# choi403/ALG

Measured on AMD Instinct MI355X. Metric: frames/sec (whole node) CogVideoX-5B-I2V 49f x 50-step ALG, higher is better.
Workload: dtype bf16; 1 GPU; BASELINE config 2: CogVideoX-5B-I2V bf16, 49 frames @ 480x720, 50 steps, ALG interval down_up (resize_factor 0.25, interval [0, 0.04]), guidance 6.0; one video per GPU; layers=42, dit_sample_forwards=12, parallelism=dp1

## Files before the change

alg_amd/_lib.py:

```python
from __future__ import annotations

import ctypes
from collections import OrderedDict
import os
from ctypes import POINTER, Structure, byref, c_char_p, c_float, c_int, c_int32, c_int64, c_void_p

import torch

_HERE = os.path.dirname(os.path.abspath(__file__))
LIB_PATH = os.environ.get("ALG_HIP_LIB") or os.path.join(_HERE, "libalg_hip.so")

ALG_F32, ALG_BF16 = 0, 1
ACT_NONE, ACT_GELU_TANH, ACT_SILU = 0, 1, 2
GEMM_BIAS_PER_ROW, GEMM_PERMUTE_COLS, GEMM_GATE_F32, GEMM_GATE_SEG_STRIDE = 1, 4, 8, 16
GEMM_B_PACKED11 = 32

EXPORTS = (
    "alg_version", "alg_last_error", "alg_reload_env", "alg_down_up", "alg_gaussian_blur", "alg_cfg_ddim_step", "alg_gemm_bf16", "alg_gemm_bf16_pair", "alg_gemm_bf16_pair_qk", "alg_pack_b_p11", "alg_pack_b_p11_bytes",
    "alg_flash_attn_d64", "alg_layernorm_modulate", "alg_layernorm_modulate_fp8", "alg_qk_norm_rope", "alg_patchify", "alg_unpatchify",
    "alg_timestep_embedding", "alg_cfg_combine", "alg_lincomb", "alg_unipc_update", "alg_concat_cast", "alg_flash_attn_d128", "alg_layernorm_mod_f32", "alg_layernorm_mod_f32_fp8", "alg_rmsnorm_rope",
    "alg_wan_modulation", "alg_patchify3d", "alg_unpatchify3d", "alg_timestep_embedding_f32", "alg_linear_f32",
    "alg_gelu_erf", "alg_layernorm_modulate_seg", "alg_headnorm_rope", "alg_masked_mean", "alg_silu", "alg_gemm_fp8", "alg_quantize_fp8_rows",
    "alg_conv_cl_bf16", "alg_vae_groupnorm_workspace", "alg_vae_groupnorm_stats", "alg_vae_spatial_norm", "alg_vae_upsample",
    "alg_vae_pack_latent", "alg_vae_unpack_video", "alg_vae_group_norm", "alg_vae_pad", "alg_vae_repitch",
    "alg_vae_unpack_planes", "alg_rms_norm_rows", "alg_softmax_hilo", "alg_flash_attn_d128_ex", "alg_flash_attn_d128_dual", "alg_rope_half", "alg_patchify_t", "alg_unpatchify_t", "alg_qk_norm_rope_scaled", "alg_flash_attn_d64_ex", "alg_embed_rows", "alg_t5_layernorm", "alg_attn_bias", "alg_mul_bf16", "alg_quick_gelu",
    "alg_lowpass_tables_bytes", "alg_lowpass_tables_build", "alg_down_up_workspace_bytes", "alg_gaussian_blur_workspace_bytes",
    "alg_flash_attn_d64_workspace_bytes", "alg_calib_mfma_bf16", "alg_wall_clock_khz", "alg_attn_clock_tap",
    "alg_flash_attn_d128_fp8", "alg_quantize_fp8_khead", "alg_quantize_fp8_vt", "alg_rmsnorm_rope_fp8", "alg_headnorm_rope_fp8",
)
_RET_I64 = ("alg_vae_groupnorm_workspace", "alg_lowpass_tables_bytes", "alg_down_up_workspace_bytes",
            "alg_gaussian_blur_workspace_bytes", "alg_flash_attn_d64_workspace_bytes", "alg_pack_b_p11_bytes")


class AlgHipError(RuntimeError):
    pass


class GemmArgs(Structure):
    _fields_ = [
        ("A", c_void_p), ("B", c_void_p), ("C", c_void_p), ("bias", c_void_p), ("R", c_void_p), ("gate", c_void_p),
        ("lda", c_int64), ("ldb", c_int64), ("ldc", c_int64), ("ldr", c_int64),
        ("strideA", c_int64), ("strideB", c_int64), ("strideC", c_int64), ("strideR", c_int64),
        ("strideGate", c_int64),
        ("M", c_int32), ("N", c_int32), ("K", c_int32), ("batch", c_int32),
        ("seg_split", c_int32), ("act", c_int32), ("flags", c_int32),
        ("gate_seg_stride", c_int64), ("perm_col0", c_int32), ("conv_cin_log2", c_int32),
        ("a_scale", c_void_p), ("b_scale", c_void_p), ("strideAScale", c_int64), ("strideBScale", c_int64),
        ("conv_wp", c_int32), ("conv_hpwp", c_int32), ("conv_kw", c_int32), ("reserved1", c_int32),
    ]


class QkNormRopeArgs(Structure):
    _fields_ = [("wq", c_void_p), ("bq", c_void_p), ("wk", c_void_p), ("bk", c_void_p), ("cos_tab", c_void_p),
                ("sin_tab", c_void_p), ("heads", c_int32), ("text_len", c_int32), ("eps", c_float),
                ("q_scale", c_float)]


class VaeGeom(Structure):
    _fields_ = [(n, c_int32) for n in ("frames", "H", "W", "C", "first_len", "seg_len", "lat_first_single", "lat_rate",
                                       "lat_scale", "lat_h", "lat_w")]


_lib = None


def build_library(verbose=False):
    import subprocess

    src = os.path.join(_HERE, "csrc")
    r = subprocess.run(["make", "-C", src, "-j8"], capture_output=True, text=True)
    if verbose or r.returncode != 0:
        print(r.stdout[-4000:])
        print(r.stderr[-4000:])
    if r.returncode != 0:
        raise AlgHipError("building libalg_hip.so failed (see output above)")
    return LIB_PATH


# ... 59 lines not shown
    lib.alg_vae_groupnorm_workspace.argtypes = [POINTER(VaeGeom)]
    lib.alg_vae_groupnorm_stats.argtypes = [c_void_p, POINTER(VaeGeom), c_float, c_void_p, c_void_p, c_void_p]
    lib.alg_vae_spatial_norm.argtypes = [c_void_p] * 6 + [POINTER(VaeGeom), c_int, c_void_p]
    lib.alg_vae_group_norm.argtypes = [c_void_p] * 5 + [POINTER(VaeGeom), c_int, c_void_p]
    lib.alg_vae_pad.argtypes = [c_void_p, c_void_p] + [c_int] * 4 + [c_void_p]
    lib.alg_vae_repitch.argtypes = [c_void_p, c_void_p] + [c_int] * 6 + [c_void_p]
    lib.alg_vae_unpack_planes.argtypes = [c_void_p, c_void_p] + [c_int] * 4 + [c_void_p]
    lib.alg_embed_rows.argtypes = [c_void_p, c_void_p, c_void_p, c_int64, c_int, c_int, c_void_p]
    lib.alg_t5_layernorm.argtypes = [c_void_p, c_void_p, c_void_p, c_int64, c_int, c_float, c_void_p]
    lib.alg_attn_bias.argtypes = [c_void_p] * 7 + [c_int, c_int, c_int, c_int, c_int64, c_int64, c_float, c_int, c_void_p]
    lib.alg_quick_gelu.argtypes = [c_void_p, c_int64, c_void_p]
    lib.alg_mul_bf16.argtypes = [c_void_p, c_void_p, c_void_p, c_int64, c_void_p]
    lib.alg_vae_upsample.argtypes = [c_void_p, c_void_p] + [c_int] * 6 + [c_void_p]
    lib.alg_vae_pack_latent.argtypes = [c_void_p, c_int64, c_int64, c_void_p, c_int, c_int, c_int, c_int, c_float, c_void_p]
    lib.alg_vae_unpack_video.argtypes = [c_void_p, c_void_p, c_int, c_int, c_int, c_int, c_void_p]
    lib.alg_quantize_fp8_rows.argtypes = [c_void_p, c_int64, c_void_p, c_void_p, c_int64, c_int, c_void_p]
    lib.alg_timestep_embedding_f32.argtypes = [c_void_p, c_void_p, c_int, c_int, c_void_p]
    lib.alg_linear_f32.argtypes = [c_void_p] * 6 + [c_int] * 4 + [c_void_p]
    lib.alg_gelu_erf.argtypes = [c_void_p, c_int64, c_void_p]
    lib.alg_unipc_update.argtypes = [c_void_p] * 5 + [c_int64] + [c_float] * 6 + [c_void_p]
    lib.alg_gemm_bf16.argtypes = [POINTER(GemmArgs), c_void_p]
    lib.alg_gemm_bf16_pair.argtypes = [POINTER(GemmArgs), POINTER(GemmArgs), c_void_p]
    lib.alg_gemm_bf16_pair_qk.argtypes = [POINTER(GemmArgs), POINTER(GemmArgs), POINTER(QkNormRopeArgs), c_void_p]
    lib.alg_flash_attn_d64.argtypes = [c_void_p, c_void_p, c_void_p, c_void_p, c_int, c_int, c_int, c_int64, c_int64,
                                       c_int64, c_int64, c_int64, c_int64, c_float, c_void_p]
    lib.alg_layernorm_modulate.argtypes = [c_void_p, c_void_p, c_void_p, c_void_p, c_void_p, c_void_p, c_int64, c_int,
                                           c_int, c_int, c_int64, c_int64, c_int, c_float, c_void_p]
    lib.alg_layernorm_modulate_fp8.argtypes = [c_void_p] * 7 + [c_int64, c_int, c_int, c_int, c_int64, c_int, c_float, c_void_p]
    lib.alg_qk_norm_rope.argtypes = [c_void_p, c_void_p, c_void_p, c_void_p, c_void_p, c_void_p, c_void_p, c_int,
                                     c_int, c_int, c_int, c_float, c_void_p]
    lib.alg_qk_norm_rope_scaled.argtypes = [c_void_p] * 7 + [c_int, c_int, c_int, c_int, c_float, c_float, c_void_p]
    lib.alg_flash_attn_d64_ex.argtypes = [c_void_p, c_void_p, c_void_p, c_void_p, c_int, c_int, c_int, c_int64, c_int64,
                                          c_int64, c_int64, c_int64, c_int64, c_float, c_int, c_void_p, c_int64, c_void_p]
    lib.alg_patchify.argtypes = [c_void_p, c_int64, POINTER(c_void_p), c_void_p, c_int, c_int, c_int, c_int, c_int,
                                 c_int, c_void_p]
    lib.alg_unpatchify.argtypes = [c_void_p, c_void_p, c_int, c_int, c_int, c_int, c_int, c_int, c_void_p]
    lib.alg_patchify_t.argtypes = [c_void_p, c_int64, POINTER(c_void_p), c_void_p] + [c_int] * 7 + [c_void_p]
    lib.alg_unpatchify_t.argtypes = [c_void_p, c_void_p] + [c_int] * 7 + [c_void_p]
    lib.alg_timestep_embedding.argtypes = [c_void_p, c_void_p, c_int, c_int, c_int, c_void_p]
    lib.alg_calib_mfma_bf16.argtypes = [c_void_p, c_int, ctypes.c_uint, c_int, c_void_p, c_void_p]
    lib.alg_attn_clock_tap.argtypes = [c_void_p, c_int]
    for name in EXPORTS:
        fn = getattr(lib, name)
        if name == "alg_attn_clock_tap":
            fn.restype = None
        elif name not in ("alg_version", "alg_last_error", "alg_reload_env"):
# ... 600 lines not shown
        _check(lib.alg_gemm_bf16(ctypes.byref(args), _stream()), "alg_gemm_bf16")


def gemm_pair(first, second):
    lib = load_library()
    a, fa = gemm_args(*first[0], **first[1])
    b, fb = gemm_args(*second[0], **second[1])
    if fa or fb:
        raise AlgHipError("gemm_pair takes bf16 problems")
    _check(lib.alg_gemm_bf16_pair(ctypes.byref(a), ctypes.byref(b), _stream()), "alg_gemm_bf16_pair")


def gemm_pair_qk(first, second, wq, bq, wk, bk, cos, sin, heads, text_len, eps, q_scale=1.0):
    lib = load_library()
    a, fa = gemm_args(*first[0], **first[1])
    b, fb = gemm_args(*second[0], **second[1])
    if fa or fb:
        raise AlgHipError("gemm_pair_qk takes bf16 problems")
    ptrs = [t.data_ptr() if t is not None else None for t in (wq, bq, wk, bk, cos, sin)]
    e = QkNormRopeArgs(*ptrs, heads, text_len, float(eps), float(q_scale))
    _check(lib.alg_gemm_bf16_pair_qk(ctypes.byref(a), ctypes.byref(b), ctypes.byref(e), _stream()), "alg_gemm_bf16_pair_qk")


def quantize_fp8_rows(x, q, scale, rows, K, x_rstride=None, x_off=0, q_off=0, scale_off=0):
    x_rstride = K if x_rstride is None else x_rstride
    _check(load_library().alg_quantize_fp8_rows(_p(x, x_off), x_rstride, _p(q, q_off), _p(scale, scale_off), rows, K,
                                                _stream()), "alg_quantize_fp8_rows")
    return q, scale


ATTN_Q_PRESCALED = 1


def flash_attn_d64(q, k, vt, o, batch, heads, S, q_bstride, q_rstride, vt_bstride, vt_rstride, o_bstride, o_rstride,
                   scale, q_off=0, k_off=0, q_prescaled=False):
    lib = load_library()
    flags = ATTN_Q_PRESCALED if q_prescaled else 0
    wsb = int(lib.alg_flash_attn_d64_workspace_bytes(batch, heads, S, flags))
    ws = scratch(o, wsb, "attn_d64")
    _check(lib.alg_flash_attn_d64_ex(c_void_p(q.data_ptr() + 2 * q_off), c_void_p(k.data_ptr() + 2 * k_off), _ptr(vt),
                                     _ptr(o), batch, heads, S, q_bstride, q_rstride, vt_bstride, vt_rstride, o_bstride,
                                     o_rstride, float(scale), flags, _ptr(ws), wsb, _stream()),
           "alg_flash_attn_d64")


def layernorm_modulate(x, y, weight, bias, scale, shift, mod_bstride, batch, rows, D, seg_split, eps,
# ... 43 lines not shown
```

alg_amd/csrc/gemm.hip:

```cpp
#include <stdlib.h>

#include "common.h"

namespace alg {
constexpr int BM = 256, BN = 256;
int launch_gemm_p6(const alg_gemm_args* a, int m_tiles, int n_tiles, int64_t nwg, hipStream_t s);
int launch_gemm_p9(const alg_gemm_args* a, int m_tiles, int n_tiles, int64_t nwg, hipStream_t s);
int launch_gemm_p9_pair(const alg_gemm_args* a, int m_tiles_a, int n_tiles_a, const alg_gemm_args* b, int m_tiles_b, int n_tiles_b,
                        hipStream_t s);
int launch_gemm_p9_pair_qk(const alg_gemm_args* a, int m_tiles_a, int n_tiles_a, const alg_gemm_args* b, int m_tiles_b, int n_tiles_b,
                           const alg_qk_norm_rope_args* e, hipStream_t s);
int launch_gemm_p10(const alg_gemm_args* a, int m_tiles, int n_tiles, int64_t nwg, hipStream_t s);
int launch_gemm_p10_pair(const alg_gemm_args* a, int m_tiles_a, int n_tiles_a, const alg_gemm_args* b, int m_tiles_b, int n_tiles_b,
                         hipStream_t s);
int launch_gemm_p10_pair_qk(const alg_gemm_args* a, int m_tiles_a, int n_tiles_a, const alg_gemm_args* b, int m_tiles_b, int n_tiles_b,
                            const alg_qk_norm_rope_args* e, hipStream_t s);
int launch_gemm_p11(const alg_gemm_args* a, int m_tiles, int n_tiles, int64_t nwg, hipStream_t s);
int launch_gemm_p6_fp8(const alg_gemm_args* a, int m_tiles, int n_tiles, int64_t nwg, hipStream_t s);
int launch_gemm_p9_fp8(const alg_gemm_args* a, int m_tiles, int n_tiles, int64_t nwg, hipStream_t s);
int launch_gemm_p6_conv(const alg_gemm_args* a, int m_tiles, int n_tiles, int64_t nwg, hipStream_t s);
static int gemm_pipe() { return opt(OPT_GEMM_PIPE); }
static bool asm_pipe() { return gemm_pipe() == 9 || gemm_pipe() == 10; }
}

using namespace alg;

static int gemm_entry(const alg_gemm_args* a, void* stream, bool fp8, bool validate_only = false) {
  if (!a || !a->A || !a->B || !a->C) {
    set_error("alg_gemm_bf16: null argument");
    return ALG_EINVAL;
  }
  if (a->M <= 0 || a->N <= 0 || a->K <= 0 || a->batch <= 0) {
    set_error("alg_gemm_bf16: bad shape M=%d N=%d K=%d batch=%d", a->M, a->N, a->K, a->batch);
    return ALG_EINVAL;
  }
  if (a->K % (fp8 ? 128 : 64) != 0) {
    set_error("alg_gemm_%s: K=%d must be a multiple of %d", fp8 ? "fp8" : "bf16", a->K, fp8 ? 128 : 64);
    return ALG_EINVAL;
  }
  const int al = fp8 ? 16 : 8;
// ... 148 lines not shown
      ((uintptr_t)e->cos_tab & 15) || ((uintptr_t)e->sin_tab & 15) || ((uintptr_t)a->C & 15)) {
    set_error("alg_gemm_bf16_pair_qk: pointers must be 16-byte aligned");
    return ALG_EINVAL;
  }
  if (a->N != 2 * e->heads * 64 || a->ldc != a->N || a->strideC != (int64_t)a->M * a->N || (a->flags & ALG_GEMM_PERMUTE_COLS) ||
      a->R || a->act != ALG_ACT_NONE) {
    set_error("alg_gemm_bf16_pair_qk: qk must be a plain GEMM onto the contiguous [batch][S][2][heads][64] tensor (N=%d heads=%d ldc=%lld)",
              a->N, e->heads, (long long)a->ldc);
    return ALG_EINVAL;
  }
  const bool fused = asm_pipe() && pair_eligible(a) && pair_eligible(b) && e->heads % 4 == 0 &&
                     !(a->bias && (a->flags & ALG_GEMM_BIAS_PER_ROW));
  if (fused) {
    const int64_t ta = (int64_t)((a->M + BM - 1) / BM) * ((a->N + BN - 1) / BN) * a->batch;
    const int64_t tb = (int64_t)((b->M + BM - 1) / BM) * ((b->N + BN - 1) / BN) * b->batch;
    if (ta + tb <= 0x7fffffff)
      return (gemm_pipe() == 10 ? launch_gemm_p10_pair_qk : launch_gemm_p9_pair_qk)(a, (a->M + BM - 1) / BM, (a->N + BN - 1) / BN, b, (b->M + BM - 1) / BM, (b->N + BN - 1) / BN, e,
                                    (hipStream_t)stream);
  }
  rc = alg_gemm_bf16_pair(a, b, stream);
  if (rc != ALG_OK) return rc;
  return alg_qk_norm_rope_scaled(a->C, e->wq, e->bq, e->wk, e->bk, e->cos_tab, e->sin_tab, a->batch, a->M, e->heads, e->text_len,
                                 e->eps, e->q_scale, stream);
}

extern "C" int alg_gemm_fp8(const alg_gemm_args* a, void* stream) { return gemm_entry(a, stream, true); }

extern "C" int alg_conv_cl_bf16(const void* x, const void* w, const void* bias, const void* res, void* y, int frames,
                                int Hp, int Wp, int Cin, int Cout, int kt, int mode, void* stream) {
  const bool pair = mode == ALG_CONV_PAIR, down = mode == ALG_CONV_STRIDE2;
  if (frames <= 0 || Hp < 3 || Wp < 3 || (kt != 1 && kt != 3) || Cin < 64 || (Cin & (Cin - 1)) || Cout <= 0 || (Cout & 3) ||
      mode < 0 || mode > ALG_CONV_STRIDE2 || (pair && (((Hp * Wp) & 1) || Cout > 128)) ||
      (down && (kt != 1 || (Hp & 1) || (Wp & 1)))) {
    set_error("alg_conv_cl_bf16: bad shape frames=%d Hp=%d Wp=%d Cin=%d Cout=%d kt=%d (Cin a power of two >= 64, Cout %% 4 == 0)",
              frames, Hp, Wp, Cin, Cout, kt);
    return ALG_EINVAL;
  }
  alg_gemm_args a = {};
  a.A = x, a.B = w, a.C = y, a.bias = bias, a.R = res;
  const int vox = pair ? 2 : 1, kw = pair ? 4 : 3;
  a.lda = (int64_t)vox * Cin, a.ldb = (int64_t)kt * 3 * kw * Cin, a.ldc = (int64_t)vox * Cout, a.ldr = a.ldc;
  a.strideA = (int64_t)Hp * Wp * Cin, a.strideB = 0, a.strideC = (int64_t)Hp * Wp * Cout, a.strideR = a.strideC;
  a.M = Hp * Wp / vox, a.N = vox * Cout, a.K = kt * 3 * kw * Cin, a.batch = frames;
  a.act = ALG_ACT_NONE;
  a.conv_cin_log2 = __builtin_ctz((unsigned)Cin), a.conv_wp = Wp, a.conv_hpwp = Hp * Wp, a.conv_kw = kw;
  if (down) {
// ... 8 lines not shown
```

alg_amd/csrc/gemm_kernel.h:

```cpp
#pragma once
#include <stdlib.h>

#include <type_traits>

#include "common.h"
#include "qk_norm_rope.h"
#ifdef ALG_P9_LOOP_INC
#include ALG_P9_LOOP_INC
#else
#include "gemm_p9_loop.inc"
#endif
#include "gemm_p9_fp8_loop.inc"
#ifdef ALG_P11_LOOP_INC
#include ALG_P11_LOOP_INC
#else
#include "gemm_p11_loop.inc"
#endif
#ifdef ALG_P10_LOOP_INC
#include ALG_P10_LOOP_INC
#else
#include "gemm_p10_loop.inc"
#endif

#ifndef ALG_FP8_MX
// ... 65 lines not shown
    return x * __builtin_amdgcn_rcpf(1.0f + __builtin_amdgcn_exp2f(x * fmaf(k2, x * x, k1)));
  }
  if (act == ALG_ACT_SILU) {
    return x * __builtin_amdgcn_rcpf(1.0f + __builtin_amdgcn_exp2f(-1.4426950408889634f * x));
  }
  return x;
}

__device__ __forceinline__ void unpack4(const uint2 v, float (&f)[4]) {
  f[0] = __uint_as_float(v.x << 16);
  f[1] = __uint_as_float(v.x & 0xffff0000u);
  f[2] = __uint_as_float(v.y << 16);
  f[3] = __uint_as_float(v.y & 0xffff0000u);
}

struct GemmNoPair {};
struct GemmPairArgs {
  alg_gemm_args p;
  int m_tiles, n_tiles, group_m;
};
struct GemmPairQkArgs : GemmPairArgs {
  QkNormRope qe;
};
template <int PAIR> struct GemmPairT { typedef GemmNoPair type; };
template <> struct GemmPairT<1> { typedef GemmPairArgs type; };
template <> struct GemmPairT<2> { typedef GemmPairQkArgs type; };
template <int ACT, bool RES, int PIPE, int WNW = 4, bool FP8 = false, bool CONV = false, int PAIR = 0>
__global__ __launch_bounds__((PIPE == 11 ? 1 : 2) * WNW * 64) void gemm_bf16_kernel(
    const alg_gemm_args p1, int m_tiles1, int n_tiles1, int group_m1, const typename GemmPairT<PAIR>::type pr) {
  constexpr bool P9 = PIPE == 9 || PIPE == 10 || PIPE == 11;
  constexpr bool M16 = PIPE == 10 || PIPE == 11;
  constexpr bool P11 = PIPE == 11;
  constexpr int WMW = P11 ? 1 : 2;
  constexpr int MT = BM / WMW / 32;
  static_assert(!PAIR || (P9 && !P11 && !RES && ACT == ALG_ACT_NONE), "the pair launch is built for the plain schedule-9 / 10 kernels");
  static_assert(!FP8 || PIPE == 6 || PIPE == 9, "the fp8 operands are built on the ping-pong schedule and on schedule 9");
  static_assert(!CONV || (PIPE == 6 && !FP8), "the convolution addressing is built on the bf16 ping-pong schedule");
  typedef typename std::conditional<FP8, uint8_t, bf16_t>::type elem_t;
  constexpr int EPS = 16 / (int)sizeof(elem_t);
  constexpr int GEMM_THREADS = WMW * WNW * 64;
  constexpr int NT = BN / WNW / 32;
  static_assert(PIPE == 0 || PIPE == 6 || PIPE == 7 || PIPE == 8 || P9,
                "schedules built: 0 (2-stage ring), 6 (ping-pong), 7 (4-wave interleaved), 8 (4-wave BK = 32 ring), 9 / 10 (asm loops)");
  static_assert((PIPE == 7 || PIPE == 8 || PIPE == 9 || PIPE == 10) == (WNW == 2) && P11 == (WNW == 4 && WMW == 1),
                "PIPE 7 / 8 / 9 / 10 are the 2 x 2 4-wave layouts, 11 the 1 x 4 one, the others run 8 waves");
  static_assert(!P11 || (!FP8 && !CONV), "schedule 11 takes bf16 plain GEMM addressing with a packed B");
  static_assert(!P9 || !CONV, "schedules 9 / 10 take plain GEMM addressing (bf16, or e4m3 on 9 since round 4)");
  constexpr bool BK64 = true;
  constexpr bool PP = PIPE == 6;
  constexpr int BK = FP8 ? 128 : 64;
  constexpr int NSTAGE = 2;
  constexpr int ROW_BYTES = BK * (int)sizeof(elem_t);
  constexpr int SLOTS = ROW_BYTES / 16;
  constexpr int TILE_BYTES = BM * ROW_BYTES;
  constexpr int STAGE_BYTES = 2 * TILE_BYTES;
  constexpr int LD_PER_OP = TILE_BYTES / (GEMM_THREADS * 16);
  constexpr int ROWS_PER_LD = GEMM_THREADS / SLOTS;
  static_assert(NSTAGE * STAGE_BYTES == GEMM_LDS, "ring must fill the 128 KiB LDS budget");

  extern __shared__ __attribute__((aligned(16))) char smem[];
  const int tid = threadIdx.x;
  const int lane = tid & 63;
  const int wave = __builtin_amdgcn_readfirstlane(tid >> 6);
  const int wm = wave / WNW, wn = wave % WNW;

  constexpr int abl = 0;
#ifdef ALG_GEMM_TAP
  uint64_t tap_loop = 0, tap_tiles = 0;
  const uint64_t tap_c0 = __builtin_readcyclecounter(), tap_r0 = wall_clock64();
#endif
  group_m1 &= 0xffff;
  const int total1 = m_tiles1 * n_tiles1 * p1.batch;
  auto do_tile = [&](const int wg_in) __attribute__((always_inline)) {
  bool second = false;
  if constexpr (PAIR) second = wg_in >= total1;
  const alg_gemm_args& p = [&]() -> const alg_gemm_args& {
    if constexpr (PAIR) return second ? pr.p : p1;
    else return p1;
  }();
  int m_tiles = m_tiles1, n_tiles = n_tiles1, group_m = group_m1, wg = wg_in;
  if constexpr (PAIR) {
    if (second) m_tiles = pr.m_tiles, n_tiles = pr.n_tiles, group_m = pr.group_m, wg = wg_in - total1;
  }
  const int tiles = m_tiles * n_tiles;
  const int b = wg / tiles;
  int t = wg - b * tiles;
  const int grp = t / (group_m * n_tiles);
  const int first_m = grp * group_m;
  const int gsize = min(m_tiles - first_m, group_m);
  t -= grp * group_m * n_tiles;
  const int m0 = (first_m + t % gsize) * BM;
  const int n0 = (t / gsize) * BN;

  const elem_t* A = (const elem_t*)p.A + (int64_t)b * p.strideA;
  const elem_t* B = (const elem_t*)p.B + (int64_t)b * p.strideB;

  const int srow = tid / SLOTS;
  const int sw_src = !BK64 ? ((tid >> 4) & 3) : ((tid >> 4) & 7);
  const int sslot = (tid & (SLOTS - 1)) ^ sw_src;
  const elem_t* a_src[LD_PER_OP];
  const elem_t* b_src[LD_PER_OP];
#pragma unroll
  for (int i = 0; i < LD_PER_OP; ++i) {
    const int r = i * ROWS_PER_LD + srow;
// ... 578 lines not shown
  const bool perm = p.flags & ALG_GEMM_PERMUTE_COLS;
  const int64_t gate_seg = (p.flags & ALG_GEMM_GATE_SEG_STRIDE) ? p.gate_seg_stride : p.N;
  const bool gate_f32 = RES && p.gate && (p.flags & ALG_GEMM_GATE_F32);
  bf16_t* Cb = (bf16_t*)p.C + (int64_t)b * p.strideC;
  const int ldc = (int)p.ldc, ldr = (int)p.ldr;
  const int col0 = perm ? p.perm_col0 : 0;
  const bool n_vec = (p.N & 3) == 0 && (col0 & 15) == 0;
  auto blk_row = [&](int mt) { return PP ? (mt >> 1) * 128 + wm * 64 + (mt & 1) * 32 : wm * (MT * 32) + mt * 32; };
  auto blk_col = [&](int nt) { return PP ? nt * 128 + wn * 32 : wn * (NT * 32) + nt * 32; };
  auto quad_row = [](int q, int ln_) { return M16 ? 16 * (q >> 1) + (ln_ & 15) : (ln_ & 31); };
  auto quad_col = [](int q, int ln_) { return M16 ? 16 * (q & 1) + 4 * (ln_ >> 4) : 8 * q + 4 * (ln_ >> 5); };
  auto rq = [](int q) { return M16 ? q >> 1 : 0; };
  auto cq = [](int q) { return M16 ? q & 1 : q; };
  constexpr int NRQ = M16 ? 2 : 1, NCQ = M16 ? 2 : 4;
  if constexpr (PP || PIPE == 8 || P9) {
    const bool staged = staged_epilogue() && ((!RES && ACT == ALG_ACT_NONE) || !(bias && bias_row));
    int lane_e = lane, l31_e = l31, h2_e = h2;
    if constexpr (P9) {
      int z = 0;
      asm volatile("" : "+s"(z));
      lane_e = __builtin_amdgcn_mbcnt_hi(~0u, __builtin_amdgcn_mbcnt_lo(~0u, z));
      l31_e = lane_e & 31, h2_e = lane_e >> 5;
    }
    if (staged) {
      char* const my = smem + wave * (MT * NT * 2048);
      constexpr bool NT_OUTER = FP8 && PIPE == 9 && RES;
      uint2 bcol[NT_OUTER ? 1 : NT][4];
      float4 scol[FP8 && !NT_OUTER ? NT : 1][FP8 && !NT_OUTER ? 4 : 1];
      float brow4[MT][NRQ], a_sc4[MT];
      if constexpr (!NT_OUTER)
#pragma unroll
      for (int nt = 0; nt < NT; ++nt)
#pragma unroll
        for (int g = 0; g < NCQ; ++g) {
          const int n = n0 + blk_col(nt) + (M16 ? quad_col(g, lane_e) : 8 * g + 4 * h2_e);
          const int nc = n < p.N ? n : 0;
          if constexpr (BIAS_EARLY) bcol[nt][g] = bcol_early[nt][g];
          else bcol[nt][g] = (bias && !bias_row) ? *(const uint2*)(bias + nc) : make_uint2(0u, 0u);
          if constexpr (FP8) scol[nt][g] = *(const float4*)(p.b_scale + (int64_t)b * p.strideBScale + nc);
        }
#pragma unroll
      for (int mt = 0; mt < MT; ++mt) {
#pragma unroll
        for (int r = 0; r < NRQ; ++r) {
          const int row = m0 + blk_row(mt) + quad_row(2 * r, lane_e);
          const int rowc = row < p.M ? row : p.M - 1;
// ... 462 lines not shown
                if (gate_f32) {
                  x = bf2f(R[rowc * ldr + nn]) +
                      ((const float*)p.gate)[(int64_t)b * p.strideGate + (seg1 ? gate_seg : 0) + nn] * x;
                } else {
                  const float gg = gate ? bf2f(gate[(seg1 ? gate_seg : 0) + nn]) : 1.0f;
                  x = bf2f(R[rowc * ldr + nn]) + rbf(gg * x);
                }
              }
              const int nj = nn + col0;
              const int nc = perm ? ((nj & ~12) | ((nj & 4) << 1) | ((nj & 8) >> 1)) : nn;
              Cb[row * ldc + nc] = f2bf(x);
            }
          }
        }
      }
    });
  };
#ifndef ALG_EPI_STAGED_ONLY
  static_for<MT>([&](auto mt_c) { epilogue_band(mt_c); });
#endif
  };

  int total_wg = total1;
  if constexpr (PAIR) total_wg += pr.m_tiles * pr.n_tiles * pr.p.batch;
  for (int L = blockIdx.x; L < total_wg; L += gridDim.x) {
    const int xcd = L & 7, q = total_wg >> 3, r = total_wg & 7;
    const int wg = (xcd < r ? xcd * (q + 1) : r * (q + 1) + (xcd - r) * q) + (L >> 3);
    if (L != (int)blockIdx.x) __syncthreads();
    do_tile(wg);
  }
#ifdef ALG_GEMM_TAP
  if (threadIdx.x == 0 && blockIdx.x < 1024) {
    uint64_t* t = gemm_tap_buf + blockIdx.x * 4;
    t[0] = __builtin_readcyclecounter() - tap_c0, t[1] = wall_clock64() - tap_r0, t[2] = tap_loop, t[3] = tap_tiles;
  }
#endif
}

inline unsigned gemm_grid(int64_t nwg) {
  static std::atomic<int> cus{0};
  int n = cus.load();
  if (n == 0) {
    hipDeviceProp_t prop;
    int dev = 0;
    n = (hipGetDevice(&dev) == hipSuccess && hipGetDeviceProperties(&prop, dev) == hipSuccess) ? prop.multiProcessorCount : 256;
    n &= ~7;
    if (n < 8) n = 8;
// ... 55 lines not shown
```

alg_amd/csrc/gemm_p11.hip:

```cpp
#include "gemm_kernel.h"

namespace alg {
int launch_gemm_p11(const alg_gemm_args* a, int m_tiles, int n_tiles, int64_t nwg, hipStream_t s) {
  return launch_gemm<11, 4>(a, m_tiles, n_tiles, nwg, s);
}

__global__ __launch_bounds__(256) void pack_b_p11_kernel(const bf16_t* __restrict__ w, uint4* __restrict__ out, int N, int K, int64_t ldb,
                                                          int64_t total) {
  const int64_t i = (int64_t)blockIdx.x * 256 + threadIdx.x;
  if (i >= total) return;
  const int lane = (int)(i & 63);
  const int f = (int)((i >> 6) & 7), wv = (int)((i >> 9) & 3);
  const int64_t tile = i >> 11;
  const int nkt = K / 64;
  const int kt = (int)(tile % nkt);
  const int64_t nt = tile / nkt;
  const int n = (int)(nt * 256) + wv * 64 + (f & 3) * 16 + (lane & 15);
  const int k = kt * 64 + (f >> 2) * 32 + (lane >> 4) * 8;
  uint4 v = make_uint4(0u, 0u, 0u, 0u);
  if (n < N) v = *(const uint4*)(w + (int64_t)n * ldb + k);
  out[i] = v;
}
}

using namespace alg;

extern "C" int64_t alg_pack_b_p11_bytes(int N, int K) {
// ... 19 lines not shown
```

alg_amd/transformer_cogvideox.py:

```python
from __future__ import annotations

import math
import os
from dataclasses import dataclass, asdict
from typing import Optional

import torch

from . import _lib


@dataclass
class CogVideoXTransformerConfig:

    num_attention_heads: int = 48
    attention_head_dim: int = 64
    in_channels: int = 32
    out_channels: int = 16
    num_layers: int = 42
    time_embed_dim: int = 512
    text_embed_dim: int = 4096
    max_text_seq_length: int = 226
    sample_width: int = 90
    sample_height: int = 60
# ... 30 lines not shown
    FP8_WEIGHTS = ("wqk", "wv", "wo", "wf1", "wf2")

    def __init__(self, config: CogVideoXTransformerConfig, weights: dict, device="cuda", fp8=False):
        cfg = self.config = config
        self.device = torch.device(device)
        if self.device.type != "cuda":
            raise _lib.AlgHipError("CogVideoXTransformer3DModel runs on the GPU only (HIP kernels, no CPU fallback)")
        if cfg.attention_head_dim != 64:
            raise _lib.AlgHipError("the attention kernel is specialised for head_dim 64")
        if cfg.ofs_embed_dim is not None and cfg.ofs_embed_dim != cfg.time_embed_dim:
            raise _lib.AlgHipError("ofs_embed_dim must equal time_embed_dim (emb = emb + ofs_emb)")
        D = cfg.inner_dim
        if D % 512:
            raise _lib.AlgHipError("inner_dim must be a multiple of 512 (LayerNorm kernel tiling)")
        self.fp8 = bool(fp8)
        if self.fp8:
            self._check_fp8_shapes()
        self.fuse_quant = True
        _lib.load_library()
        self.attn_prescale = True
        self.pair_qkv = True
        self.fuse_qk_norm = False
        self.packed_weights = True
        self._sincos = {}
        dev = self.device
        w = weights
        p = cfg.patch_size
        self.p_t = cfg.patch_size_t or 1
        self.k_patch = cfg.in_channels * p * p * self.p_t
        if self.k_patch % 64 or cfg.text_embed_dim % 64 or cfg.time_embed_dim % 64:
            raise _lib.AlgHipError("GEMM K dimensions must be multiples of 64")
        self.w_patch = _bf(w["patch_embed.proj.weight"].reshape(D, self.k_patch), dev)
        self.b_patch = _bf(w["patch_embed.proj.bias"], dev)
        self.w_text = _bf(w["patch_embed.text_proj.weight"], dev)
        self.b_text = _bf(w["patch_embed.text_proj.bias"], dev)
        self.pos_emb = _bf(w["patch_embed.pos_embedding"][0], dev) if cfg.use_learned_positional_embeddings else None
        self.w_t1 = _bf(w["time_embedding.linear_1.weight"], dev)
        self.b_t1 = _bf(w["time_embedding.linear_1.bias"], dev)
        self.w_t2 = _bf(w["time_embedding.linear_2.weight"], dev)
        self.b_t2 = _bf(w["time_embedding.linear_2.bias"], dev)
        if cfg.ofs_embed_dim is not None:
            self.w_o1, self.b_o1 = _bf(w["ofs_embedding.linear_1.weight"], dev), _bf(w["ofs_embedding.linear_1.bias"], dev)
            self.w_o2, self.b_o2 = _bf(w["ofs_embedding.linear_2.weight"], dev), _bf(w["ofs_embedding.linear_2.bias"], dev)

        def reorder6(t):
            c = t.chunk(6, dim=0)
# ... 7 lines not shown
            for nm in ("norm1", "norm2"):
                mw.append(reorder6(w[b + nm + ".linear.weight"]))
                mb.append(reorder6(w[b + nm + ".linear.bias"]))
                L[nm + "_w"] = _bf(w[b + nm + ".norm.weight"], dev)
                L[nm + "_b"] = _bf(w[b + nm + ".norm.bias"], dev)
            L["wqk"] = _bf(torch.cat([w[b + "attn1.to_q.weight"], w[b + "attn1.to_k.weight"]], dim=0), dev)
            L["bqk"] = _bf(torch.cat([w[b + "attn1.to_q.bias"], w[b + "attn1.to_k.bias"]], dim=0), dev)
            L["wv"] = _bf(w[b + "attn1.to_v.weight"], dev)
            L["bv"] = _bf(w[b + "attn1.to_v.bias"], dev)
            for nm in ("norm_q", "norm_k"):
                L[nm + "_w"] = _bf(w[b + "attn1." + nm + ".weight"], dev)
                L[nm + "_b"] = _bf(w[b + "attn1." + nm + ".bias"], dev)
            L["wo"] = _bf(w[b + "attn1.to_out.0.weight"], dev)
            L["bo"] = _bf(w[b + "attn1.to_out.0.bias"], dev)
            L["wf1"] = _bf(w[b + "ff.net.0.proj.weight"], dev)
            L["bf1"] = _bf(w[b + "ff.net.0.proj.bias"], dev)
            L["wf2"] = _bf(w[b + "ff.net.2.weight"], dev)
            L["bf2"] = _bf(w[b + "ff.net.2.bias"], dev)
            if self.fp8:
                self._quantize_layer(L, drop_bf16=True)
            else:
                for nm in ("wo", "wf1", "wf2"):
                    L["p" + nm] = _lib.PackedB(L[nm])
            self.layers.append(L)
        ow, ob = w["norm_out.linear.weight"], w["norm_out.linear.bias"]
        sh_w, sc_w = ow.chunk(2, dim=0)
        sh_b, sc_b = ob.chunk(2, dim=0)
        mw.append(torch.cat([sh_w, sh_w, sc_w, sc_w], dim=0))
        mb.append(torch.cat([sh_b, sh_b, sc_b, sc_b], dim=0))
        self.w_mod = _bf(torch.cat(mw, dim=0), dev)
        self.b_mod = _bf(torch.cat(mb, dim=0), dev)
        self.mod_cols = self.w_mod.shape[0]
        self.norm_final_w = _bf(w["norm_final.weight"], dev)
        self.norm_final_b = _bf(w["norm_final.bias"], dev)
        self.norm_out_w = _bf(w["norm_out.norm.weight"], dev)
        self.norm_out_b = _bf(w["norm_out.norm.bias"], dev)
        self.w_out = _bf(w["proj_out.weight"], dev)
        self.b_out = _bf(w["proj_out.bias"], dev)
        self._ws = {}
        self._rope_cache = {}
        self.profile = None

    def _check_fp8_shapes(self):
        cfg = self.config
        D, F4 = cfg.inner_dim, cfg.ff_inner_mult * cfg.inner_dim
        if D % 128 or F4 % 128:
# ... 228 lines not shown
            emb, osin, o1, oemb = (torch.empty(N, E, device=self.device, dtype=torch.bfloat16) for _ in range(4))
            G(ws["t1"], self.w_t2, emb, N, E, E, E, E, E, bias=self.b_t2)
            ofs_v = ofs.to(device=self.device, dtype=torch.float32).reshape(-1)
            ofs_v = (ofs_v if ofs_v.numel() == N else ofs_v[:1].expand(N)).contiguous()
            _lib.timestep_embedding(ofs_v, osin, N, O, cfg.flip_sin_to_cos)
            G(osin, self.w_o1, o1, N, O, O, O, O, O, bias=self.b_o1, act=_lib.ACT_SILU)
            G(o1, self.w_o2, oemb, N, O, O, O, O, O, bias=self.b_o2)
            _lib.lincomb([(1.0, emb), (1.0, oemb)], torch.bfloat16, out=emb)
            _lib.silu(emb, ws["semb"])
        G(ws["semb"], self.w_mod, mod, N, self.mod_cols, E, E, E, self.mod_cols, bias=self.b_mod)

        G(ehs, self.w_text, x, T, D, cfg.text_embed_dim, cfg.text_embed_dim, cfg.text_embed_dim, D,
          bias=self.b_text, R=pos_emb, ldr=D, batch=N, strideA=T * cfg.text_embed_dim, strideC=S * D)
        _lib.patchify(lat, 0 if Bl == 1 else Fr * C * Hh * Ww, conds, ws["patches"], N, Fr, C, Hh, Ww, p, p_t)
        G(ws["patches"], self.w_patch, x, P, D, self.k_patch, self.k_patch, self.k_patch, D, bias=self.b_patch,
          R=pos_emb, ldr=D, r_off=T * D, batch=N, strideA=P * self.k_patch, strideC=S * D, c_off=T * D)

        scale = 1.0 / math.sqrt(cfg.attention_head_dim)
        prescale = self.attn_prescale
        q_scale = scale * 1.4426950408889634 if prescale else 1.0
        F4 = cfg.ff_inner_mult * D
        packed = self.packed_weights and os.environ.get("ALG_GEMM_PIPE", "10") == "10"
        wo_k, wf1_k, wf2_k = ("pwo", "pwf1", "pwf2") if packed else ("wo", "wf1", "wf2")
        for li, L in enumerate(self.layers):
            m1 = li * 12 * D
            m2 = m1 + 6 * D
            if fp8:
                self._block_fp8(L, ws, q8, q8s, N, S, T, m1, m2, cos, sin, scale, q_scale, prescale)
                continue
            TM("ln_mod", _lib.layernorm_modulate, x, y, L["norm1_w"], L["norm1_b"], mod, mod, self.mod_cols, N, S, D,
               T, cfg.norm_eps, scale_off=m1 + 2 * D, shift_off=m1)
            qk_call = ((y, L["wqk"], qk, S, 2 * D, D, D, D, 2 * D), dict(bias=L["bqk"], batch=N, strideA=S * D, strideC=S * 2 * D))
            vt_call = ((L["wv"], y, vt, D, S, D, D, D, S_pad), dict(bias=L["bv"], batch=N, strideB=S * D, strideC=D * S_pad,
                                                                   flags=_lib.GEMM_BIAS_PER_ROW | _lib.GEMM_PERMUTE_COLS))
            if self.pair_qkv and self.fuse_qk_norm:
                TM("gemm_qkv", _lib.gemm_pair_qk, qk_call, vt_call, L["norm_q_w"], L["norm_q_b"], L["norm_k_w"], L["norm_k_b"], cos, sin,
                               Hn, T, cfg.qk_norm_eps, q_scale=q_scale)
            else:
                if self.pair_qkv:
                    TM("gemm_qkv", _lib.gemm_pair, qk_call, vt_call)
                else:
                    TM("gemm_qk", G, *qk_call[0], **qk_call[1])
                    TM("gemm_vt", G, *vt_call[0], **vt_call[1])
                TM("qk_norm_rope", _lib.qk_norm_rope_, qk, L["norm_q_w"], L["norm_q_b"], L["norm_k_w"], L["norm_k_b"], cos, sin, N, S, Hn, T,
                                   cfg.qk_norm_eps, q_scale=q_scale)
            TM("attn", _lib.flash_attn_d64, qk, qk, vt, att, N, Hn, S, S * 2 * D, 2 * D, D * S_pad, S_pad, S * D, D, scale,
                                k_off=D, q_prescaled=prescale)
            TM("gemm_out", G, att, L[wo_k], x, S, D, D, D, D, D, bias=L["bo"], R=x, ldr=D, gate=mod, gate_off=m1 + 4 * D,
              strideGate=self.mod_cols, seg_split=T, batch=N, strideA=S * D, strideC=S * D, strideR=S * D)
            TM("ln_mod", _lib.layernorm_modulate, x, y, L["norm2_w"], L["norm2_b"], mod, mod, self.mod_cols, N, S, D,
               T, cfg.norm_eps, scale_off=m2 + 2 * D, shift_off=m2)
            TM("gemm_ff1", G, y, L[wf1_k], h, S, F4, D, D, D, F4, bias=L["bf1"], act=_lib.ACT_GELU_TANH, batch=N, strideA=S * D,
              strideC=S * F4)
            TM("gemm_ff2", G, h, L[wf2_k], x, S, D, F4, F4, F4, D, bias=L["bf2"], R=x, ldr=D, gate=mod, gate_off=m2 + 4 * D,
              strideGate=self.mod_cols, seg_split=T, batch=N, strideA=S * F4, strideC=S * D, strideR=S * D)

        _lib.layernorm_modulate(x, y, self.norm_final_w, self.norm_final_b, None, None, 0, N, S, D, T, cfg.norm_eps)
        mo = cfg.num_layers * 12 * D
# ... 26 lines not shown
```

include/alg_hip.h:

```cpp
#ifndef ALG_HIP_H
#define ALG_HIP_H

#include <stdint.h>

#ifdef __cplusplus
extern "C" {
#endif

#define ALG_F32 0
#define ALG_BF16 1

#define ALG_OK 0
#define ALG_EINVAL (-1)
#define ALG_ELAUNCH (-2)
#define ALG_ELIMIT (-3)

#define ALG_VERSION 110

int alg_version(void);
const char* alg_last_error(void);

void alg_reload_env(void);


// ... 57 lines not shown
  const float* b_scale;
  int64_t strideAScale, strideBScale;
  int32_t conv_wp;
  int32_t conv_hpwp;
  int32_t conv_kw;
  int32_t reserved1;
} alg_gemm_args;

int alg_gemm_bf16(const alg_gemm_args* args, void* stream);

int64_t alg_pack_b_p11_bytes(int N, int K);
int alg_pack_b_p11(const void* w, void* packed, int N, int K, int64_t ldb, void* stream);

int alg_gemm_bf16_pair(const alg_gemm_args* a, const alg_gemm_args* b, void* stream);

typedef struct alg_qk_norm_rope_args {
  const void *wq, *bq, *wk, *bk;
  const float *cos_tab, *sin_tab;
  int32_t heads, text_len;
  float eps, q_scale;
} alg_qk_norm_rope_args;
int alg_gemm_bf16_pair_qk(const alg_gemm_args* qk, const alg_gemm_args* vt, const alg_qk_norm_rope_args* e, void* stream);

int alg_gemm_fp8(const alg_gemm_args* args, void* stream);

int alg_quantize_fp8_rows(const void* x, int64_t x_rstride, void* q, float* scale, int64_t rows, int K, void* stream);

int alg_flash_attn_d64(const void* q, const void* k, const void* vt, void* o, int batch, int heads, int S,
                       int64_t q_bstride, int64_t q_rstride, int64_t vt_bstride, int64_t vt_rstride,
                       int64_t o_bstride, int64_t o_rstride, float scale, void* stream);

#define ALG_ATTN_Q_PRESCALED 1
int alg_flash_attn_d64_ex(const void* q, const void* k, const void* vt, void* o, int batch, int heads, int S,
                          int64_t q_bstride, int64_t q_rstride, int64_t vt_bstride, int64_t vt_rstride,
                          int64_t o_bstride, int64_t o_rstride, float scale, int flags, void* workspace,
                          int64_t workspace_bytes, void* stream);
int64_t alg_flash_attn_d64_workspace_bytes(int batch, int heads, int S, int flags);

int alg_flash_attn_d128(const void* q, const void* k, const void* vt, void* o, int batch, int heads, int Sq, int Skv,
                        int64_t q_bstride, int64_t q_rstride, int64_t k_bstride, int64_t k_rstride, int64_t vt_bstride,
                        int64_t vt_rstride, int64_t o_bstride, int64_t o_rstride, float scale, void* stream);

int alg_flash_attn_d128_ex(const void* q, const void* k, const void* vt, void* o, int batch, int heads, int Sq, int Skv,
                           int64_t q_bstride, int64_t q_rstride, int64_t k_bstride, int64_t k_rstride, int64_t vt_bstride,
                           int64_t vt_rstride, int64_t o_bstride, int64_t o_rstride, float scale, int kv_group, int causal,
                           void* stream);
// ... 160 lines not shown
```

Baseline: 1.501 frames/s.

## Fold QKV projections into one packed GEMM with a transposing V epilogue

Concatenates the QK and V weights into one packed-B matrix and runs a single schedule-11 GEMM over N=3D. Column tiles at or beyond n_split take a new epilogue that goes through LDS and writes V transposed and column-permuted into the vt buffer that attention reads. This replaces the paired schedule-10 QK/VT launch with the packed schedule-11 kernel and avoids reading the activation twice. In exchange it adds a complex shuffle epilogue and extra weight memory for the concatenated packed copy, and it only applies under the default pipe.

```diff
diff --git a/alg_amd/_lib.py b/alg_amd/_lib.py
--- a/alg_amd/_lib.py
+++ b/alg_amd/_lib.py
@@ -16,7 +16,7 @@
 GEMM_B_PACKED11 = 32
 
 EXPORTS = (
-    "alg_version", "alg_last_error", "alg_reload_env", "alg_down_up", "alg_gaussian_blur", "alg_cfg_ddim_step", "alg_gemm_bf16", "alg_gemm_bf16_pair", "alg_gemm_bf16_pair_qk", "alg_pack_b_p11", "alg_pack_b_p11_bytes",
+    "alg_version", "alg_last_error", "alg_reload_env", "alg_down_up", "alg_gaussian_blur", "alg_cfg_ddim_step", "alg_gemm_bf16", "alg_gemm_bf16_pair", "alg_gemm_bf16_pair_qk", "alg_gemm_bf16_split_t", "alg_pack_b_p11", "alg_pack_b_p11_bytes",
     "alg_flash_attn_d64", "alg_layernorm_modulate", "alg_layernorm_modulate_fp8", "alg_qk_norm_rope", "alg_patchify", "alg_unpatchify",
     "alg_timestep_embedding", "alg_cfg_combine", "alg_lincomb", "alg_unipc_update", "alg_concat_cast", "alg_flash_attn_d128", "alg_layernorm_mod_f32", "alg_layernorm_mod_f32_fp8", "alg_rmsnorm_rope",
     "alg_wan_modulation", "alg_patchify3d", "alg_unpatchify3d", "alg_timestep_embedding_f32", "alg_linear_f32",
@@ -54,6 +54,10 @@
     _fields_ = [("wq", c_void_p), ("bq", c_void_p), ("wk", c_void_p), ("bk", c_void_p), ("cos_tab", c_void_p),
                 ("sin_tab", c_void_p), ("heads", c_int32), ("text_len", c_int32), ("eps", c_float),
                 ("q_scale", c_float)]
+
+
+class GemmSplitTArgs(Structure):
+    _fields_ = [("Ct", c_void_p), ("ldct", c_int64), ("strideCt", c_int64), ("n_split", c_int32), ("perm_col0", c_int32)]
 
 
 class VaeGeom(Structure):
@@ -159,6 +163,7 @@
     lib.alg_gemm_bf16.argtypes = [POINTER(GemmArgs), c_void_p]
     lib.alg_gemm_bf16_pair.argtypes = [POINTER(GemmArgs), POINTER(GemmArgs), c_void_p]
     lib.alg_gemm_bf16_pair_qk.argtypes = [POINTER(GemmArgs), POINTER(GemmArgs), POINTER(QkNormRopeArgs), c_void_p]
+    lib.alg_gemm_bf16_split_t.argtypes = [POINTER(GemmArgs), POINTER(GemmSplitTArgs), c_void_p]
     lib.alg_flash_attn_d64.argtypes = [c_void_p, c_void_p, c_void_p, c_void_p, c_int, c_int, c_int, c_int64, c_int64,
                                        c_int64, c_int64, c_int64, c_int64, c_float, c_void_p]
     lib.alg_layernorm_modulate.argtypes = [c_void_p, c_void_p, c_void_p, c_void_p, c_void_p, c_void_p, c_int64, c_int,
@@ -805,6 +810,15 @@
     _check(lib.alg_gemm_bf16_pair_qk(ctypes.byref(a), ctypes.byref(b), ctypes.byref(e), _stream()), "alg_gemm_bf16_pair_qk")
 
 
+def gemm_split_t(problem, n_split, Ct, ldct, strideCt=0, perm_col0=0, ct_off=0):
+    lib = load_library()
+    a, fp8 = gemm_args(*problem[0], **problem[1])
+    if fp8:
+        raise AlgHipError("gemm_split_t takes a bf16 problem")
+    t = GemmSplitTArgs((Ct.data_ptr() + 2 * ct_off) if Ct is not None else None, ldct, strideCt, n_split, perm_col0)
+    _check(lib.alg_gemm_bf16_split_t(ctypes.byref(a), ctypes.byref(t), _stream()), "alg_gemm_bf16_split_t")
+
+
 def quantize_fp8_rows(x, q, scale, rows, K, x_rstride=None, x_off=0, q_off=0, scale_off=0):
     x_rstride = K if x_rstride is None else x_rstride
     _check(load_library().alg_quantize_fp8_rows(_p(x, x_off), x_rstride, _p(q, q_off), _p(scale, scale_off), rows, K,
diff --git a/alg_amd/csrc/gemm.hip b/alg_amd/csrc/gemm.hip
--- a/alg_amd/csrc/gemm.hip
+++ b/alg_amd/csrc/gemm.hip
@@ -16,6 +16,7 @@
 int launch_gemm_p10_pair_qk(const alg_gemm_args* a, int m_tiles_a, int n_tiles_a, const alg_gemm_args* b, int m_tiles_b, int n_tiles_b,
                             const alg_qk_norm_rope_args* e, hipStream_t s);
 int launch_gemm_p11(const alg_gemm_args* a, int m_tiles, int n_tiles, int64_t nwg, hipStream_t s);
+int launch_gemm_p11_split_t(const alg_gemm_args* a, int m_tiles, int n_tiles, int64_t nwg, const alg_gemm_split_t_args* t, hipStream_t s);
 int launch_gemm_p6_fp8(const alg_gemm_args* a, int m_tiles, int n_tiles, int64_t nwg, hipStream_t s);
 int launch_gemm_p9_fp8(const alg_gemm_args* a, int m_tiles, int n_tiles, int64_t nwg, hipStream_t s);
 int launch_gemm_p6_conv(const alg_gemm_args* a, int m_tiles, int n_tiles, int64_t nwg, hipStream_t s);
@@ -210,6 +211,50 @@
   if (rc != ALG_OK) return rc;
   return alg_qk_norm_rope_scaled(a->C, e->wq, e->bq, e->wk, e->bk, e->cos_tab, e->sin_tab, a->batch, a->M, e->heads, e->text_len,
                                  e->eps, e->q_scale, stream);
+}
+
+extern "C" int alg_gemm_bf16_split_t(const alg_gemm_args* a, const alg_gemm_split_t_args* t, void* stream) {
+  const int rc = gemm_entry(a, stream, false, true);
+  if (rc != ALG_OK) return rc;
+  if (!t) {
+    set_error("alg_gemm_bf16_split_t: null argument");
+    return ALG_EINVAL;
+  }
+  if (!(a->flags & ALG_GEMM_B_PACKED11) || (a->flags & ~ALG_GEMM_B_PACKED11) || a->R || a->gate || a->act != ALG_ACT_NONE || a->a_scale ||
+      a->b_scale || a->conv_wp || a->conv_cin_log2 || a->conv_kw) {
+    set_error("alg_gemm_bf16_split_t: takes a plain bf16 problem with a packed B (ALG_GEMM_B_PACKED11 and no other flag; no residual, gate, "
+              "activation, e4m3 scales or convolution addressing)");
+    return ALG_EINVAL;
+  }
+  if (gemm_pipe() != 10) {
+    set_error("alg_gemm_bf16_split_t: built for the default schedule only (ALG_GEMM_PIPE=%d): run the two projections as their own calls", gemm_pipe());
+    return ALG_EINVAL;
+  }
+  if (t->n_split < 0 || t->n_split % BN || t->n_split > a->N) {
+    set_error("alg_gemm_bf16_split_t: n_split=%d must be a multiple of %d in [0, N=%d]", t->n_split, BN, a->N);
+    return ALG_EINVAL;
+  }
+  if ((a->N & 7) || (a->ldc & 7) || (a->strideC & 7) || ((uintptr_t)a->C & 15) || a->ldc < t->n_split) {
+    set_error("alg_gemm_bf16_split_t: N %% 8 == 0, C 16-byte aligned with ldc / strideC multiples of 8 and ldc >= n_split (N=%d ldc=%lld)", a->N,
+              (long long)a->ldc);
+    return ALG_EINVAL;
+  }
+  if (t->n_split < a->N) {
+    const int64_t m16 = ((int64_t)a->M + 15) / 16 * 16;
+    if (!t->Ct || ((uintptr_t)t->Ct & 15) || (t->ldct & 7) || (t->strideCt & 7) || t->perm_col0 < 0 || (t->perm_col0 & 15) ||
+        t->ldct < t->perm_col0 + m16) {
+      set_error("alg_gemm_bf16_split_t: Ct 16-byte aligned, ldct / strideCt multiples of 8, perm_col0 a multiple of 16, ldct >= perm_col0 + M "
+                "rounded up to 16 (M=%d ldct=%lld perm_col0=%d)", a->M, (long long)t->ldct, t->perm_col0);
+      return ALG_EINVAL;
+    }
+  }
+  const int m_tiles = (a->M + BM - 1) / BM, n_tiles = (a->N + BN - 1) / BN;
+  const int64_t nwg = (int64_t)m_tiles * n_tiles * a->batch;
+  if ((int64_t)a->M * a->ldc >= (1ll << 31) || nwg > 0x7fffffff) {
+    set_error("alg_gemm_bf16_split_t: M*ldc must stay below 2^31 (32-bit epilogue offsets; this entry does not cut slabs)");
+    return ALG_ELIMIT;
+  }
+  return launch_gemm_p11_split_t(a, m_tiles, n_tiles, nwg, t, (hipStream_t)stream);
 }
 
 extern "C" int alg_gemm_fp8(const alg_gemm_args* a, void* stream) { return gemm_entry(a, stream, true); }
diff --git a/alg_amd/csrc/gemm_kernel.h b/alg_amd/csrc/gemm_kernel.h
--- a/alg_amd/csrc/gemm_kernel.h
+++ b/alg_amd/csrc/gemm_kernel.h
@@ -111,9 +111,15 @@
 struct GemmPairQkArgs : GemmPairArgs {
   QkNormRope qe;
 };
+struct GemmSplitT {
+  bf16_t* Ct;
+  int64_t ldct, strideCt;
+  int n_split, col0;
+};
 template <int PAIR> struct GemmPairT { typedef GemmNoPair type; };
 template <> struct GemmPairT<1> { typedef GemmPairArgs type; };
 template <> struct GemmPairT<2> { typedef GemmPairQkArgs type; };
+template <> struct GemmPairT<3> { typedef GemmSplitT type; };
 template <int ACT, bool RES, int PIPE, int WNW = 4, bool FP8 = false, bool CONV = false, int PAIR = 0>
 __global__ __launch_bounds__((PIPE == 11 ? 1 : 2) * WNW * 64) void gemm_bf16_kernel(
     const alg_gemm_args p1, int m_tiles1, int n_tiles1, int group_m1, const typename GemmPairT<PAIR>::type pr) {
@@ -122,7 +128,10 @@
   constexpr bool P11 = PIPE == 11;
   constexpr int WMW = P11 ? 1 : 2;
   constexpr int MT = BM / WMW / 32;
-  static_assert(!PAIR || (P9 && !P11 && !RES && ACT == ALG_ACT_NONE), "the pair launch is built for the plain schedule-9 / 10 kernels");
+  constexpr bool PAIRED = PAIR == 1 || PAIR == 2;
+  constexpr bool SPLIT_T = PAIR == 3;
+  static_assert(!PAIRED || (P9 && !P11 && !RES && ACT == ALG_ACT_NONE), "the pair launch is built for the plain schedule-9 / 10 kernels");
+  static_assert(!SPLIT_T || (P11 && !RES && ACT == ALG_ACT_NONE), "the transposing exit is built for the plain schedule-11 kernel");
   static_assert(!FP8 || PIPE == 6 || PIPE == 9, "the fp8 operands are built on the ping-pong schedule and on schedule 9");
   static_assert(!CONV || (PIPE == 6 && !FP8), "the convolution addressing is built on the bf16 ping-pong schedule");
   typedef typename std::conditional<FP8, uint8_t, bf16_t>::type elem_t;
@@ -162,13 +171,13 @@
   const int total1 = m_tiles1 * n_tiles1 * p1.batch;
   auto do_tile = [&](const int wg_in) __attribute__((always_inline)) {
   bool second = false;
-  if constexpr (PAIR) second = wg_in >= total1;
+  if constexpr (PAIRED) second = wg_in >= total1;
   const alg_gemm_args& p = [&]() -> const alg_gemm_args& {
-    if constexpr (PAIR) return second ? pr.p : p1;
+    if constexpr (PAIRED) return second ? pr.p : p1;
     else return p1;
   }();
   int m_tiles = m_tiles1, n_tiles = n_tiles1, group_m = group_m1, wg = wg_in;
-  if constexpr (PAIR) {
+  if constexpr (PAIRED) {
     if (second) m_tiles = pr.m_tiles, n_tiles = pr.n_tiles, group_m = pr.group_m, wg = wg_in - total1;
   }
   const int tiles = m_tiles * n_tiles;
@@ -793,6 +802,79 @@
       lane_e = __builtin_amdgcn_mbcnt_hi(~0u, __builtin_amdgcn_mbcnt_lo(~0u, z));
       l31_e = lane_e & 31, h2_e = lane_e >> 5;
     }
+    if constexpr (SPLIT_T) {
+      if (n0 >= pr.n_split) {
+        char* const my = smem + wave * 32768;
+        const int odd = lane_e & 1;
+        const int lm = lane_e & 14, lmp = (lm & ~12) | ((lm & 4) << 1) | ((lm & 8) >> 1);
+        const int nl = 4 * (lane_e >> 4) + 2 * odd;
+        const int swl = ((nl >> 1) & 7) << 1;
+        char* const wbase = my + nl * 512 + (lmp & 7) * 2;
+        float bvt[NT][2][4];
+#pragma unroll
+        for (int nt = 0; nt < NT; ++nt)
+#pragma unroll
+          for (int g = 0; g < 2; ++g) unpack4(bcol_early[nt][g], bvt[nt][g]);
+        __builtin_amdgcn_sched_barrier(0);
+        static_for<MT>([&](auto mt_c) {
+          constexpr int mt = decltype(mt_c)::value;
+          static_for<NT>([&](auto nt_c) {
+            constexpr int nt = decltype(nt_c)::value;
+            const f32x16 blk = get_acc(mt_c, nt_c);
+#pragma unroll
+            for (int g = 0; g < 4; ++g) {
+              float v[4];
+#pragma unroll
+              for (int i = 0; i < 4; ++i) v[i] = blk[4 * g + i] + bvt[nt][g & 1][i];
+              const uint32_t ox = pack_bf2(v[0], v[1]), oy = pack_bf2(v[2], v[3]);
+              const uint32_t recv = (uint32_t)__builtin_amdgcn_mov_dpp((int)(odd ? ox : oy), 0xb1, 0xf, 0xf, true);
+              const uint32_t mine = odd ? oy : ox;
+              const uint32_t lo = odd ? recv : mine, hi = odd ? mine : recv;
+              const uint32_t w0 = (lo & 0xffffu) | (hi << 16), w1 = (lo >> 16) | (hi & 0xffff0000u);
+              const int chunk = ((mt * 4 + 2 * (g >> 1)) ^ swl) | (lmp >> 3);
+              char* const wp = wbase + (nt * 32 + 16 * (g & 1)) * 512 + chunk * 16;
+              *(uint32_t*)wp = w0;
+              *(uint32_t*)(wp + 512) = w1;
+            }
+          });
+        });
+        asm volatile("s_waitcnt lgkmcnt(0)" ::: "memory");
+        bf16_t* const Ctb = pr.Ct + (int64_t)b * pr.strideCt + pr.col0 + m0;
+        const int nrow0 = n0 - pr.n_split + wn * 64;
+        const int c_l = lane_e & 31, r_l = lane_e >> 5;
+        const int src_hi = m0 + (c_l >> 1) * 16 + ((c_l & 1) ? 15 : 11);
+        const bool full = src_hi < p.M;
+        static_for<4>([&](auto grp_c) {
+          constexpr int g0 = decltype(grp_c)::value * 8;
+          uint4 raw[8];
+          static_for<8>([&](auto j_c) {
+            constexpr int it = g0 + decltype(j_c)::value;
+            raw[decltype(j_c)::value] = *(const uint4*)(my + (2 * it + r_l) * 512 + ((c_l ^ ((it & 7) << 1)) * 16));
+          });
+          static_for<8>([&](auto j_c) {
+            constexpr int it = g0 + decltype(j_c)::value;
+            const int nr = 2 * it + r_l;
+            if (pr.n_split + nrow0 + nr < p.N) {
+              bf16_t* const dst = Ctb + (int64_t)(nrow0 + nr) * pr.ldct + c_l * 8;
+              const uint4 outv = raw[decltype(j_c)::value];
+              if (full) {
+                ALG_STORE16(dst, outv);
+              } else {
+                const uint32_t u[4] = {outv.x, outv.y, outv.z, outv.w};
+#pragma unroll
+                for (int e = 0; e < 8; ++e) {
+                  const int pos = c_l * 8 + e;
+                  const int src = m0 + ((pos & ~12) | ((pos & 4) << 1) | ((pos & 8) >> 1));
+                  if (src < p.M) dst[e] = (bf16_t)((e & 1) ? (u[e >> 1] >> 16) : (u[e >> 1] & 0xffffu));
+                }
+              }
+            }
+          });
+          __builtin_amdgcn_sched_barrier(0);
+        });
+        return;
+      }
+    }
     if (staged) {
       char* const my = smem + wave * (MT * NT * 2048);
       constexpr bool NT_OUTER = FP8 && PIPE == 9 && RES;
@@ -1301,7 +1383,7 @@
   };
 
   int total_wg = total1;
-  if constexpr (PAIR) total_wg += pr.m_tiles * pr.n_tiles * pr.p.batch;
+  if constexpr (PAIRED) total_wg += pr.m_tiles * pr.n_tiles * pr.p.batch;
   for (int L = blockIdx.x; L < total_wg; L += gridDim.x) {
     const int xcd = L & 7, q = total_wg >> 3, r = total_wg & 7;
     const int wg = (xcd < r ? xcd * (q + 1) : r * (q + 1) + (xcd - r) * q) + (L >> 3);
diff --git a/alg_amd/csrc/gemm_p11.hip b/alg_amd/csrc/gemm_p11.hip
--- a/alg_amd/csrc/gemm_p11.hip
+++ b/alg_amd/csrc/gemm_p11.hip
@@ -3,6 +3,25 @@
 namespace alg {
 int launch_gemm_p11(const alg_gemm_args* a, int m_tiles, int n_tiles, int64_t nwg, hipStream_t s) {
   return launch_gemm<11, 4>(a, m_tiles, n_tiles, nwg, s);
+}
+
+int launch_gemm_p11_split_t(const alg_gemm_args* a, int m_tiles, int n_tiles, int64_t nwg, const alg_gemm_split_t_args* t, hipStream_t s) {
+  const void* fn = (const void*)gemm_bf16_kernel<ALG_ACT_NONE, false, 11, 4, false, false, 3>;
+  static PerDeviceOnce attr_set;
+  const int dev_slot = current_device_slot();
+  if (!device_done(attr_set, dev_slot)) {
+    hipError_t e = hipFuncSetAttribute(fn, hipFuncAttributeMaxDynamicSharedMemorySize, GEMM_LDS_P9);
+    if (e != hipSuccess) {
+      set_error("alg_gemm_bf16_split_t: hipFuncSetAttribute(%d B LDS): %s", GEMM_LDS_P9, hipGetErrorString(e));
+      return ALG_ELAUNCH;
+    }
+    device_mark(attr_set, dev_slot);
+  }
+  GemmSplitT sp;
+  sp.Ct = (bf16_t*)t->Ct, sp.ldct = t->ldct, sp.strideCt = t->strideCt, sp.n_split = t->n_split, sp.col0 = t->perm_col0;
+  hipLaunchKernelGGL((gemm_bf16_kernel<ALG_ACT_NONE, false, 11, 4, false, false, 3>), dim3(gemm_grid(nwg)), dim3(256), GEMM_LDS_P9, s, *a,
+                     m_tiles, n_tiles, gemm_group_m(11, n_tiles, a->K), sp);
+  return check_launch("alg_gemm_bf16_split_t");
 }
 
 __global__ __launch_bounds__(256) void pack_b_p11_kernel(const bf16_t* __restrict__ w, uint4* __restrict__ out, int N, int K, int64_t ldb,
diff --git a/alg_amd/transformer_cogvideox.py b/alg_amd/transformer_cogvideox.py
--- a/alg_amd/transformer_cogvideox.py
+++ b/alg_amd/transformer_cogvideox.py
@@ -76,6 +76,7 @@
         self.pair_qkv = True
         self.fuse_qk_norm = False
         self.packed_weights = True
+        self.fold_qkv = True
         self._sincos = {}
         dev = self.device
         w = weights
@@ -129,6 +130,8 @@
             else:
                 for nm in ("wo", "wf1", "wf2"):
                     L["p" + nm] = _lib.PackedB(L[nm])
+                L["pwqkv"] = _lib.PackedB(torch.cat([L["wqk"], L["wv"]], dim=0))
+                L["bqkv"] = torch.cat([L["bqk"], L["bv"]], dim=0)
             self.layers.append(L)
         ow, ob = w["norm_out.linear.weight"], w["norm_out.linear.bias"]
         sh_w, sc_w = ow.chunk(2, dim=0)
@@ -403,6 +406,7 @@
         F4 = cfg.ff_inner_mult * D
         packed = self.packed_weights and os.environ.get("ALG_GEMM_PIPE", "10") == "10"
         wo_k, wf1_k, wf2_k = ("pwo", "pwf1", "pwf2") if packed else ("wo", "wf1", "wf2")
+        fold = bool(packed and self.fold_qkv and self.pair_qkv and not self.fuse_qk_norm and self.layers and "pwqkv" in self.layers[0])
         for li, L in enumerate(self.layers):
             m1 = li * 12 * D
             m2 = m1 + 6 * D
@@ -414,7 +418,13 @@
             qk_call = ((y, L["wqk"], qk, S, 2 * D, D, D, D, 2 * D), dict(bias=L["bqk"], batch=N, strideA=S * D, strideC=S * 2 * D))
             vt_call = ((L["wv"], y, vt, D, S, D, D, D, S_pad), dict(bias=L["bv"], batch=N, strideB=S * D, strideC=D * S_pad,
                                                                    flags=_lib.GEMM_BIAS_PER_ROW | _lib.GEMM_PERMUTE_COLS))
-            if self.pair_qkv and self.fuse_qk_norm:
+            if fold:
+                TM("gemm_qkv", _lib.gemm_split_t, ((y, L["pwqkv"], qk, S, 3 * D, D, D, D, 2 * D),
+                                                   dict(bias=L["bqkv"], batch=N, strideA=S * D, strideC=S * 2 * D)),
+                   2 * D, vt, S_pad, strideCt=D * S_pad)
+                TM("qk_norm_rope", _lib.qk_norm_rope_, qk, L["norm_q_w"], L["norm_q_b"], L["norm_k_w"], L["norm_k_b"], cos, sin, N, S, Hn, T,
+                                   cfg.qk_norm_eps, q_scale=q_scale)
+            elif self.pair_qkv and self.fuse_qk_norm:
                 TM("gemm_qkv", _lib.gemm_pair_qk, qk_call, vt_call, L["norm_q_w"], L["norm_q_b"], L["norm_k_w"], L["norm_k_b"], cos, sin,
                                Hn, T, cfg.qk_norm_eps, q_scale=q_scale)
             else:
diff --git a/include/alg_hip.h b/include/alg_hip.h
--- a/include/alg_hip.h
+++ b/include/alg_hip.h
@@ -103,6 +103,14 @@
 } alg_qk_norm_rope_args;
 int alg_gemm_bf16_pair_qk(const alg_gemm_args* qk, const alg_gemm_args* vt, const alg_qk_norm_rope_args* e, void* stream);
 
+typedef struct alg_gemm_split_t_args {
+  void* Ct;
+  int64_t ldct, strideCt;
+  int32_t n_split;
+  int32_t perm_col0;
+} alg_gemm_split_t_args;
+int alg_gemm_bf16_split_t(const alg_gemm_args* args, const alg_gemm_split_t_args* t, void* stream);
+
 int alg_gemm_fp8(const alg_gemm_args* args, void* stream);
 
 int alg_quantize_fp8_rows(const void* x, int64_t x_rstride, void* q, float* scale, int64_t rows, int K, void* stream);
```

New measurement: 1.512 frames/s, median of 6. No clear change (+0.7%).
